# jolibrain/jolineedle

Measured on AMD Instinct MI355X. Metric: glimpse-patches/sec (448px, seq-len 20) REINFORCE step, higher is better.
Workload: dtype f32; 1 GPU; configs[2]/[3]: REINFORCE rollout, gpt-nano + yolox-nano encoder, 448px, seq-len 20, --enable-stop, 64 agents/GPU x 1 GPU, 4480x4480 synthetic images, forced non-STOP actions (S=T); global_batch=64, seq_len=20

## Files before the change

include/jnroll.h:

```cpp
#ifndef JNROLL_H
#define JNROLL_H

#include <stddef.h>
#include <stdint.h>

#ifdef __cplusplus
extern "C" {
#endif

#define JN_ABI_VERSION 2

enum {
  JN_OK = 0,
  JN_EINVAL = -1,
  JN_ENOMEM = -2,
  JN_EHIP = -3,
  JN_ENOTFOUND = -4,
  JN_ESTATE = -5
};

enum { JN_MODE_GREEDY = 0, JN_MODE_SAMPLE = 1, JN_MODE_FORCED = 2 };

enum { JN_NET_GPT_BACKBONE = 0, JN_NET_DETECTOR = 1 };

// ... 117 lines not shown
int jn_gather_patches_views(const jn_image_view* views_dev, int n_views, const int64_t* image_index_dev,
                            const int64_t* positions_dev, void* out_dev, int out_u8, int N, int Hc, int Wc, int P,
                            void* stream);

#define JN_AUG_NPARAM 20
int jn_augment_patches(const float* in_dev, float* out_dev, const float* params_dev, const float* noise_dev,
                       uint64_t seed, int N, int P, void* stream);

int jn_backbone_forward(jn_ctx* ctx, int net, const float* patches_dev, int N, int train,
                        float* fpn0_dev, float* fpn1_dev, float* fpn2_dev, void* stream);
int jn_read_tensor(jn_ctx* ctx, const char* name, float* host_out, size_t numel);
int jn_embed_patches(jn_ctx* ctx, const float* patches_dev, int N, float* out_dev, void* stream);
int jn_zero_grad(jn_ctx* ctx, void* stream);
int jn_backbone_backward(jn_ctx* ctx, int net, const float* patches_dev, int N, const float* g0_dev,
                         const float* g1_dev, const float* g2_dev, void* stream);
typedef struct jn_train_opts {
  int32_t struct_size;
  int32_t reward_norm;
  float ret_mean, ret_std;
  float entropy_weight;
  float loss_scale;
} jn_train_opts;

int jn_reinforce_step(jn_ctx* ctx, int mode, const int64_t* forced_actions_dev,
                      const int64_t* start_positions_dev, uint64_t seed, int stop_early,
                      const jn_train_opts* opts, const jn_rollout_out* out, float* metrics_dev, void* stream);
int jn_reinforce_forward(jn_ctx* ctx, int mode, const int64_t* forced_actions_dev, const int64_t* start_positions_dev,
                         uint64_t seed, int stop_early, const jn_rollout_out* out, void* stream);
int jn_reinforce_backward(jn_ctx* ctx, const float* dlogprobs_dev, const float* dentropies_dev, void* stream);
int jn_arena_segment(jn_ctx* ctx, const char* name, size_t* off, size_t* numel);
// ... 53 lines not shown
```

jolineedle_amd/_lib.py:

```python
import ctypes as C
import os
from pathlib import Path

_LIB = None
LIB_PATH = Path(__file__).resolve().parent / "lib" / "libjnroll.so"

JN_MODE_GREEDY, JN_MODE_SAMPLE, JN_MODE_FORCED = 0, 1, 2
JN_NET_GPT_BACKBONE, JN_NET_DETECTOR = 0, 1


class LibraryNotBuilt(RuntimeError):
    pass


class JnError(RuntimeError):
    pass


class JnConfig(C.Structure):
    _fields_ = [("struct_size", C.c_int32), ("device", C.c_int32),
                ("n_layer", C.c_int32), ("n_head", C.c_int32), ("n_embd", C.c_int32),
                ("block_size", C.c_int32), ("n_actions", C.c_int32), ("patch_size", C.c_int32),
                ("use_pos_emb", C.c_int32), ("no_patch_emb", C.c_int32), ("concat_emb", C.c_int32),
                ("decoder_pos_encoding", C.c_int32), ("pos_emb_size", C.c_int32),
# ... 108 lines not shown
    "jn_set_profiling": (C.c_int, [C.c_void_p, C.c_int]),
    "jn_detector_step": (C.c_int, [C.c_void_p, C.c_void_p, C.c_int, C.c_void_p, C.c_int, C.c_float, C.c_void_p, C.c_void_p]),
    "jn_detector_forward": (C.c_int, [C.c_void_p, C.c_void_p, C.c_int, C.c_void_p, C.c_int, C.c_int, C.c_int, C.c_void_p,
                                      C.c_void_p, C.c_void_p, C.c_void_p, C.c_void_p, C.c_void_p, C.c_void_p]),
    "jn_detector_backward": (C.c_int, [C.c_void_p, C.c_int, C.c_void_p, C.c_float, C.c_void_p]),
    "jn_optimizer_step_group": (C.c_int, [C.c_void_p, C.c_int, C.c_float, C.c_float, C.c_float, C.c_float, C.c_void_p]),
    "jn_reinforce_forward": (C.c_int, [C.c_void_p, C.c_int, C.c_void_p, C.c_void_p, C.c_uint64, C.c_int,
                                       C.POINTER(JnRolloutOut), C.c_void_p]),
    "jn_reinforce_backward": (C.c_int, [C.c_void_p, C.c_void_p, C.c_void_p, C.c_void_p]),
    "jn_arena_segment": (C.c_int, [C.c_void_p, C.c_char_p, C.POINTER(C.c_size_t), C.POINTER(C.c_size_t)]),
    "jn_export_arena": (C.c_int, [C.c_void_p, C.c_int, C.c_void_p, C.c_size_t, C.c_int, C.c_void_p]),
    "jn_import_arena": (C.c_int, [C.c_void_p, C.c_int, C.c_void_p, C.c_size_t, C.c_void_p]),
    "jn_set_dropout": (C.c_int, [C.c_void_p, C.c_float, C.c_uint64]),
    "jn_set_freeze": (C.c_int, [C.c_void_p, C.c_int]),
    "jn_optimizer_steps": (C.c_int, [C.c_void_p, C.c_int, C.POINTER(C.c_int), C.c_int]),
}


def load_library(path=None):
    global _LIB
    if _LIB is not None and path is None:
        return _LIB
    p = Path(path or os.environ.get("JNROLL_LIB", LIB_PATH))
    if not p.exists():
        raise LibraryNotBuilt(
            f"{p} not found: the HIP extension is not built. Run `bash jolineedle_amd/csrc/build.sh` "
            "(or __graft_entry__.build()). There is no CPU fallback for this path.")
    lib = C.CDLL(str(p))
    for name, (res, args) in SIGNATURES.items():
        fn = getattr(lib, name)
# ... 22 lines not shown
```

jolineedle_amd/csrc/api.hip:

```cpp
#include <algorithm>
#include <cmath>
#include <cstdarg>
#include <cstring>
#include <memory>
#include <set>

#include "jn_internal.h"

namespace jnr {

static thread_local char g_err[512] = "";

void set_error(const char* fmt, ...) {
  va_list ap;
  va_start(ap, fmt);
  vsnprintf(g_err, sizeof(g_err), fmt, ap);
  va_end(ap);
}

int build_pafpn(Net& net, std::vector<ParamEntry>& params, const std::string& prefix, float depth, float width,
                bool depthwise, int P);
int build_head(Net& net, std::vector<ParamEntry>& params, const std::string& prefix, float width, bool depthwise,
               int num_classes);

// ... 913 lines not shown
  }
  return JN_OK;
}

static inline float* grad_of(const jn_ctx* ctx, const float* param) { return ctx->grads + (param - ctx->params); }

static int ensure_aux_stream(jn_ctx* ctx) {
  if (ctx->aux_stream) return JN_OK;
  JN_HIP(hipStreamCreateWithFlags(&ctx->aux_stream, hipStreamNonBlocking));
  JN_HIP(hipEventCreateWithFlags(&ctx->aux_fork, hipEventDisableTiming));
  JN_HIP(hipEventCreateWithFlags(&ctx->aux_join, hipEventDisableTiming));
  return JN_OK;
}

static int run_net_backward(jn_ctx* ctx, int ni, int N, const StemSrc& ss, int slot, hipStream_t s, int nsl = 1,
                            long long pos_slot_stride = 0, bool with_head = false, int fpn_zero = 0) {
  Net& net = ctx->nets[ni];
  const int MB = ctx->cfg.max_batch;
  JN_CHECK(nsl >= 1 && nsl <= net.g_slots && slot + nsl <= net.n_slots, JN_ESTATE, "backward over %d slots from %d: not allocated", nsl, slot);
  std::vector<BwdStep> plan;
  int rc = plan_backward(net, with_head, fpn_zero, plan);
  if (rc) return rc;
  JN_HIP(hipMemsetAsync(net.bred, 0, (size_t)nsl * JN_NREP * 2 * net.stat_channels * sizeof(double), s));
  const long long rep_stride = 2LL * net.stat_channels;
  SlotBatch sb;
  sb.n = nsl;
  sb.act = (long long)net.per_image_floats * MB;
  sb.grad = (long long)net.per_image_floats * MB;
  sb.tab = 3LL * net.tab_channels;
  sb.save = 2LL * net.stat_channels;
  sb.red = (long long)JN_NREP * 2 * net.stat_channels;
  sb.consts = 3LL * net.stat_channels;
  sb.pos = pos_slot_stride;
  float* save = slot_save(net, slot);
  auto ptr = [&](const View& v) { return view_ptr(net, slot, MB, v); };
  auto gptr = [&](const View& v) { return net.gact + net.buf_off[v.buf] * (size_t)MB + v.coff; };
  auto tab = [&](const View& v) { return view_tab(net, slot, v); };
  auto ld = [&](const View& v) { return net.bufs[v.buf].C; };
  auto sums = [&](int p, int half) {
    const ConvW& pcw = net.convs[net.ops[p].wslot];
    return net.bred + 2 * (pcw.stat_off + (half > 0 ? pcw.cout / 2 : 0));
  };
  const ChanTab ident{ctx->ident, ctx->ident + 2048, ctx->ident + 4096};
  static const bool no_aux = std::getenv("JN_NO_AUX_STREAM") != nullptr;
  static const bool dbg_plan = std::getenv("JN_DBG_BWD_PLAN") != nullptr;
  bool aux_used = false;
  if (!no_aux) { int ra = ensure_aux_stream(ctx); if (ra) return ra; }
  const int n_ops_b = (int)plan.size();
  static const bool bwd_profile = std::getenv("JN_BWD_PROFILE") != nullptr;
  std::vector<hipEvent_t> bev;
  if (bwd_profile) {
    bev.resize(n_ops_b + 1);
    for (auto& e : bev) (void)hipEventCreate(&e);
    (void)hipEventRecord(bev[n_ops_b], s);
  }
  for (int obi = n_ops_b - 1; obi >= 0; --obi) {
    const Op& op = net.ops[obi];
    const BwdStep& st = plan[obi];
    if (op.wslot >= 0) {
      const ConvW& cw = net.convs[op.wslot];
      float* const gp_out = gptr(st.g);
      const int gld_out = ld(st.g);
      const long long M = (long long)N * op.out.H * op.out.W;
      double* red = net.bred + 2 * cw.stat_off;
      float* consts = net.bconsts + 3 * cw.stat_off;
      const bool pair_halves = st.red_by && !cw.prefix2.empty();
      if (dbg_plan) {
        const int hm = st.red_by;
        const long long sep = pair_halves ? (M / N) * (cw.cout / 2) * (2 - ((hm & 1) + ((hm >> 1) & 1))) : hm ? 0 : (M / N) * cw.cout;
        std::fprintf(stderr, "[bwd-plan] %-34s kind %d cout %4d cin %4d M/patch %6lld stride %d acc_in %d separate-reduce elements/patch %8lld%s\n",
                     op.name.c_str(), (int)op.kind, cw.cout, cw.cin, M / N, op.stride, (int)op.acc_in, sep,
                     pair_halves ? (hm == 3 ? " (both halves by their consumers)" : " (one half by its consumer)") : "");
      }
      if (pair_halves) {
        const int h = cw.cout / 2;
        for (int half = 0; half < 2; ++half) {
          const int c0 = half * h;
          ChanTab ot = tab(op.out);
          ot.sc += c0; ot.sh += c0; ot.fl += c0;
          if (!(st.red_by & (1 << half)))
            launch_bn_bwd_reduce(gp_out + c0, gld_out, (const float*)ptr(op.out) + c0, net.act_dtype, ld(op.out), ot,
                                 save + 2 * (cw.stat_off + c0), h, M, red + 2 * c0, rep_stride, s, sb);
          launch_bn_bwd_consts(red + 2 * c0, rep_stride, (double)M, cw.gamma_dev + c0, cw.beta_dev + c0, save + 2 * (cw.stat_off + c0), consts + 3 * c0,
                               grad_of(ctx, cw.gamma_dev) + c0, grad_of(ctx, cw.beta_dev) + c0, h, s, sb, (st.red_by >> half) & 1);
        }
      } else {
        if (!st.red_by)
// ... 28 lines not shown
            const ChanTab zt = tab(co.out);
            fa.red2_z = (const float*)ptr(co.out); fa.red2_ld = ld(co.out); fa.red2_sc = zt.sc; fa.red2_sh = zt.sh;
          }
          launch_pw_bwd_fused(fa, s);
        }
      } else if (st.route == BR_DW_FUSED) {
        DwBwdFusedArgs fa{};
        fa.g = gp_out; fa.g_ld = gld_out; fa.z = (const float*)ptr(op.out); fa.z_ld = ld(op.out); fa.ot = tab(op.out);
        fa.save = save + 2 * cw.stat_off; fa.consts = consts;
        fa.x = (const float*)ptr(op.in); fa.x_ld = ld(op.in); fa.it = tab(op.in); fa.w = cw.w_dev;
        fa.gin = gptr(op.in); fa.gin_ld = ld(op.in); fa.accumulate = op.acc_in ? 1 : 0; fa.gw = gw; fa.wpart = ctx->wpart;
        fa.C = cw.cout; fa.H = op.in.H; fa.W = op.in.W; fa.OH = op.out.H; fa.OW = op.out.W; fa.N = N; fa.stride = op.stride;
        fa.sb = sb;
        if (st.red_in >= 0) {
          fa.red_in = sums(st.red_in, st.red_half); fa.red_rep_stride = rep_stride;
          fa.accumulate = 0;
        }
        launch_dw_bwd_fused(fa, s);
      } else if (st.route == BR_STEM_FUSED) {
        StemArgs a{ss.src, ss.positions, ss.pos_stride, ss.sample_stride, ss.chan_stride, ss.row_stride, net.P, N, cw.cout,
                   cw.w_dev, nullptr, 0, JN_F32, nullptr, 0, nullptr, 0, 0, ss.src_u8};
        launch_stem_bwd_weight(a, gp_out, gld_out, gw, ctx->wpart, s, sb, (const float*)ptr(op.out), ld(op.out),
                               tab(op.out), save + 2 * cw.stat_off, consts);
      } else {
        launch_bn_bwd_gz(gp_out, gld_out, ptr(op.out), net.act_dtype, ld(op.out), tab(op.out), save + 2 * cw.stat_off, consts,
                         cw.cout, M, s, sb);
        if (st.route == BR_PW) {
          ConvArgs a{};
          a.in = gp_out; a.in_ld = gld_out; a.in_dtype = JN_F32; a.itab = ident; a.w = cw.w_dev; a.bias = nullptr;
          a.out = gptr(op.in); a.out_ld = ld(op.in); a.out_dtype = JN_F32; a.bf16_mfma = net.act_dtype == JN_BF16;
          a.N = N; a.H = op.out.H; a.W = op.out.W; a.OH = op.out.H; a.OW = op.out.W;
// ... 1187 lines not shown
  launch_pw_bwd_weight(e, K, dpe, JN_F32, C, ident, grad_of(ctx, g.efpn_lin_wt), nullptr, Mr, K, C, s);
  launch_colsum_add(dpe, Mr, C, grad_of(ctx, g.efpn_lin_b), s);
  SlotBatch sb;
  sb.n = g_n; sb.act = g_slot; sb.grad = g_slot; sb.tab = 3LL * net.tab_channels;
  ConvArgs a{};
  a.in = ctx->de_ws; a.in_ld = C; a.in_dtype = JN_F32; a.itab = ident; a.w = g.efpn_w; a.bias = nullptr;
  a.out = net.gact + net.buf_off[f2.buf] * (size_t)MB + f2.coff; a.out_ld = net.bufs[f2.buf].C; a.out_dtype = JN_F32; a.bf16_mfma = 0;
  a.N = rows; a.H = f2.H; a.W = f2.W; a.OH = f2.H; a.OW = f2.W; a.cin = C; a.cout = f2.C; a.stride = 1; a.act = ACT_NONE;
  a.accumulate = 0; a.w_transposed = 1; a.in_identity = 1;
  a.n_slots = g_n; a.in_slot_stride = (long long)rows * K; a.out_slot_stride = g_slot; a.tab_slot_stride = 0;
  const bool detached = ctx->enc_net == JN_NET_DETECTOR;
  if (!detached) launch_pw(a, s);
  launch_pw_bwd_weight(ctx->de_ws, C, view_ptr(net, slot, MB, f2), net.act_dtype, net.bufs[f2.buf].C, view_tab(net, slot, f2),
                       grad_of(ctx, g.efpn_w), ctx->wpart, (long long)rows * HW, C, f2.C, s, sb, (long long)rows * K);
  if (detached) return JN_OK;
  for (int i = 0; i < 2; ++i) {
    const View& f = net.fpn[i];
    for (int j = 0; j < g_n; ++j)
      JN_HIP(hipMemsetAsync(net.gact + (size_t)j * g_slot + net.buf_off[f.buf] * (size_t)MB + f.coff, 0,
                            (size_t)rows * f.H * f.W * f.C * sizeof(float), s));
  }
  return run_net_backward(ctx, ctx->enc_net, rows, ss, slot, s, g_n, pos_slot_stride, false, 0x3);
}

}
static int reinforce_backward_impl(jn_ctx* ctx, const jn_rollout_out* out, int S, int stop_early, hipStream_t s);
static int check_train_outputs(jn_ctx* ctx, const jn_rollout_out* out) {
  JN_CHECK(out->logits_dev && out->actions_dev && out->returns_dev && out->logit_masks_dev && out->positions_dev &&
               out->final_emb_dev && out->rewards_dev && out->masks_dev,
           JN_EINVAL, "training needs logits/actions/returns/logit_masks/positions/final_emb/rewards/masks outputs");
  JN_CHECK(!ctx->cfg.no_patch_emb, JN_ESTATE, "training without a patch encoder is not supported");
  JN_CHECK(ctx->cfg.block_size <= 62, JN_EINVAL, "training supports block_size <= 62");
  JN_CHECK(ctx->cfg.act_dtype == JN_F32, JN_ESTATE, "training needs act_dtype = fp32 (bf16 is the inference mode)");
  return JN_OK;
}
extern "C" {

// ... 258 lines not shown

int jn_export_arena(jn_ctx* ctx, int what, float* dst_dev, size_t numel, int accumulate, void* stream) {
  return arena_copy(ctx, what, dst_dev, numel, 1, accumulate, stream);
}

int jn_import_arena(jn_ctx* ctx, int what, const float* src_dev, size_t numel, void* stream) {
  return arena_copy(ctx, what, const_cast<float*>(src_dev), numel, 0, 0, stream);
}

int jn_set_freeze(jn_ctx* ctx, int freeze_detector_backbone) {
  JN_CHECK(ctx, JN_EINVAL, "null ctx");
  ctx->freeze_det_backbone = freeze_detector_backbone != 0;
  return JN_OK;
}

int jn_optimizer_steps(jn_ctx* ctx, int group, int* steps, int set) {
  JN_CHECK(ctx && steps && (group == 0 || group == 1), JN_EINVAL, "jn_optimizer_steps: bad argument");
  int& st = group == 0 ? ctx->adam_step : ctx->adam_step_yolox;
  if (set) st = *steps; else *steps = st;
  return JN_OK;
}

int jn_set_dropout(jn_ctx* ctx, float p, uint64_t seed) {
  JN_CHECK(ctx && p >= 0.0f && p < 1.0f, JN_EINVAL, "dropout probability must be in [0, 1)");
  ctx->pdrop = p; ctx->drop_seed = seed; ctx->drop_ctr = 0;
  return JN_OK;
}

int jn_read_param(jn_ctx* ctx, const char* name, float* host_out, size_t numel) {
  JN_CHECK(ctx && name && host_out && ctx->params, JN_EINVAL, "jn_read_param: bad argument");
// ... 52 lines not shown
```

jolineedle_amd/csrc/jn_internal.h:

```cpp
#pragma once
#include <hip/hip_runtime.h>

#include <cstdint>
#include <cstdio>
#include <map>
#include <string>
#include <vector>

#include "../../include/jnroll.h"
#include "jn_kernels.h"

namespace jnr {

void set_error(const char* fmt, ...);

#define JN_HIP(call)                                                                      \
  do {                                                                                    \
    hipError_t e_ = (call);                                                               \
    if (e_ != hipSuccess) {                                                               \
      jnr::set_error("%s failed: %s (%s:%d)", #call, hipGetErrorString(e_), __FILE__, __LINE__); \
      return JN_EHIP;                                                                     \
    }                                                                                     \
  } while (0)

// ... 98 lines not shown

enum BwdRoute {
  BR_NONE = 0,
  BR_PW_FUSED, BR_PW_FUSED_HALVES,
  BR_DW_FUSED, BR_STEM_FUSED,
  BR_PW, BR_DW, BR_STEM, BR_CONV3_S1, BR_CONV3_S2,
  BR_ADDACT_COPY, BR_ADDACT_FOLD,
  BR_SPP, BR_UPSAMPLE,
};
struct BwdStep {
  BwdRoute route = BR_NONE;
  View g;
  int red_by = 0;
  int red_in = -1, red_half = -1, red_in2 = -1, red_half2 = -1, red_split = 0;
  bool red2 = false;
  int fold = -1;
};
int plan_backward(const Net& net, bool with_head, int fpn_zero, std::vector<BwdStep>& plan);

struct ParamEntry {
  jn_param_info info;
};

struct ParamSeg {
  std::string name;
  int kind = 0, d0 = 0, d1 = 0, d2 = 0;
  size_t off = 0, numel = 0;
};

struct GptW {
  float *wte = nullptr, *wpe = nullptr, *embed_class = nullptr;
  float *proj_wt = nullptr, *proj_b = nullptr;
  float *pos1d = nullptr;
// ... 113 lines not shown
```

jolineedle_amd/csrc/kernels_bwd.hip:

```cpp
#include <hip/hip_runtime.h>

#include <algorithm>
#include <cstdlib>
#include <type_traits>

#include "jn_kernels.h"
#include "jn_reduce.h"
#include "jn_types.h"

namespace jnr {

__device__ __forceinline__ float sigmoidf_(float v) { return __builtin_amdgcn_rcpf(1.0f + __expf(-v)); }
__device__ __forceinline__ float silu_(float v) { return v * sigmoidf_(v); }
__device__ __forceinline__ float dsilu_(float y) {
  const float s = sigmoidf_(y);
  return s * (1.0f + y * (1.0f - s));
}
__device__ __forceinline__ f32x4 tf4_(f32x4 z, f32x4 sc, f32x4 sh, f32x4 fl) {
  f32x4 r;
  r.x = fl.x != 0.0f ? silu_(fmaf(z.x, sc.x, sh.x)) : z.x;
  r.y = fl.y != 0.0f ? silu_(fmaf(z.y, sc.y, sh.y)) : z.y;
  r.z = fl.z != 0.0f ? silu_(fmaf(z.z, sc.z, sh.z)) : z.z;
  r.w = fl.w != 0.0f ? silu_(fmaf(z.w, sc.w, sh.w)) : z.w;
  return r;
// ... 888 lines not shown
  if (nb > cap) nb = cap;
  const dim3 blocks((unsigned)nb, sb.n);
  const size_t smem = (size_t)9 * C * sizeof(float);
#define JN_DWW(S_, T_)                                                                                            \
  hipLaunchKernelGGL((dw_bwd_weight_kernel<S_, T_>), blocks, dim3(256), smem, s, gz, g_ld, (const T_*)x, x_ld, it, \
                     gw, rep, C, H, W, OH, OW, N, sb)
  if (x_dtype == JN_BF16) { if (stride == 1) JN_DWW(1, bf16_t); else JN_DWW(2, bf16_t); }
  else { if (stride == 1) JN_DWW(1, float); else JN_DWW(2, float); }
#undef JN_DWW
  if (rep) launch_wpart_reduce(gw_final, wpart, 9 * C, s);
  return 0;
}

constexpr int DF_TW = 16;

template <int S, int CB, int DF_TH, bool RED>
__global__ __launch_bounds__(256) __attribute__((amdgpu_waves_per_eu(3))) void dw_bwd_fused_kernel(
    const float* __restrict__ g, int g_ld, const float* __restrict__ z, int z_ld, ChanTab ot,
    const float* __restrict__ save, const float* __restrict__ consts, const float* __restrict__ x, int x_ld,
    ChanTab it, const float* __restrict__ w, float* __restrict__ gin, int gin_ld, int accumulate,
    float* __restrict__ gw, int rep, int C, int H, int W, int OH, int OW, int tiles_x, int tiles_y, int n_tiles,
    SlotBatch sb, double* __restrict__ red_in, long long red_rep_stride) {
  constexpr int Q = CB / 4, PS = S == 1 ? CB : CB + JN_DW_S2_PAD;
  constexpr int GH = S == 1 ? DF_TH + 2 : DF_TH + 1, GW = S == 1 ? DF_TW + 2 : DF_TW + 1;
  constexpr int AH = S == 1 ? DF_TH + 2 : 2 * DF_TH + 1, AW = S == 1 ? DF_TW + 2 : 2 * DF_TW + 1;
  constexpr int GROUPS = 256 / (DF_TW * Q), RPG = DF_TH / GROUPS;
  static_assert(RPG >= 1 && RPG * GROUPS == DF_TH, "tile / thread mapping");
  extern __shared__ __attribute__((aligned(16))) float sm[];
  float* Gs = sm;
  float* As = Gs + GH * GW * PS;
  float* red = As + AH * AW * PS;
// ... 25 lines not shown
  f32x4 r1 = {0.f, 0.f, 0.f, 0.f}, r2 = {0.f, 0.f, 0.f, 0.f};
  auto reduce_in = [&](const f32x4& zv, const f32x4& dx) {
    const f32x4 i_sc = JN_C4(7), i_sh = JN_C4(8);
#pragma unroll
    for (int k = 0; k < 4; ++k) {
      const float yv = fmaf(zv[k], i_sc[k], i_sh[k]);
      const float gy = dx[k] * dsilu_(yv);
      r1[k] += gy;
      r2[k] += gy * yv;
    }
  };
  const int xx = (tid / Q) % DF_TW, grp = tid / (Q * DF_TW), j0 = grp * RPG;
  const int wg = blockIdx.x / ncb, n_wg = gridDim.x / ncb;
  constexpr bool OWNER = S == 2 && RED;
  static_assert(!OWNER || RPG == 1, "owner staging: one output pixel per thread and tile");
  f32x4 zraw[OWNER ? 4 : 1];
  for (int tile = wg; tile < n_tiles; tile += n_wg) {
    const int tx = tile % tiles_x, ty = (tile / tiles_x) % tiles_y, n = tile / (tiles_x * tiles_y);
    const int oy0 = ty * DF_TH, ox0 = tx * DF_TW;
    const int gy0 = S == 1 ? oy0 - 1 : oy0, gx0 = S == 1 ? ox0 - 1 : ox0;
    const int ay0 = oy0 * S - 1, ax0 = ox0 * S - 1;
    __syncthreads();
    for (int i = tid; i < GH * GW * Q; i += 256) {
      const int p = i / Q, r = p / GW, cx = p - r * GW;
      const int oy = gy0 + r, ox = gx0 + cx;
      f32x4 v = {0.f, 0.f, 0.f, 0.f};
      if (oy >= 0 && oy < OH && ox >= 0 && ox < OW) {
        const long long pix = ((long long)n * OH + oy) * OW + ox;
        const f32x4 gv = *reinterpret_cast<const f32x4*>(g + pix * g_ld + c);
        const f32x4 zv = *reinterpret_cast<const f32x4*>(z + pix * z_ld + c);
// ... 34 lines not shown
        const int p = i / Q, r = p / AW, cx = p - r * AW;
        const int iy = ay0 + r, ix = ax0 + cx;
        f32x4 v = {0.f, 0.f, 0.f, 0.f};
        if (iy >= 0 && iy < H && ix >= 0 && ix < W)
          v = tf4_(*reinterpret_cast<const f32x4*>(x + (((long long)n * H + iy) * W + ix) * x_ld + c), JN_C4(7), JN_C4(8), JN_C4(9));
        *reinterpret_cast<f32x4*>(As + p * PS + 4 * q) = v;
      }
    }
    __syncthreads();
#pragma unroll 1
    for (int j = 0; j < RPG; ++j) {
      const int y = j0 + j;
      if (S == 1) {
        const f32x4 gc = *reinterpret_cast<const f32x4*>(Gs + ((y + 1) * GW + xx + 1) * PS + 4 * q);
        f32x4 zin = {0.f, 0.f, 0.f, 0.f};
        if (RED && oy0 + y < H && ox0 + xx < W)
          zin = *reinterpret_cast<const f32x4*>(x + (((long long)n * H + oy0 + y) * W + ox0 + xx) * x_ld + c);
        f32x4 acc = {0.f, 0.f, 0.f, 0.f};
#pragma unroll
        for (int ky = 0; ky < 3; ++ky)
#pragma unroll
          for (int kx = 0; kx < 3; ++kx) {
            acc += *reinterpret_cast<const f32x4*>(Gs + ((y + 2 - ky) * GW + xx + 2 - kx) * PS + 4 * q) * JN_C4(10 + ky * 3 + kx);
            dw[ky * 3 + kx] += gc * *reinterpret_cast<const f32x4*>(As + ((y + ky) * AW + xx + kx) * PS + 4 * q);
          }
        const int iy = oy0 + y, ix = ox0 + xx;
        if (iy < H && ix < W) {
          float* op = gin + (((long long)n * H + iy) * W + ix) * gin_ld + c;
          if (RED) reduce_in(zin, acc);
          if (accumulate) acc += *reinterpret_cast<const f32x4*>(op);
          *reinterpret_cast<f32x4*>(op) = acc;
        }
      } else {
        const f32x4 g00 = *reinterpret_cast<const f32x4*>(Gs + (y * GW + xx) * PS + 4 * q);
        const f32x4 g01 = *reinterpret_cast<const f32x4*>(Gs + (y * GW + xx + 1) * PS + 4 * q);
        const f32x4 g10 = *reinterpret_cast<const f32x4*>(Gs + ((y + 1) * GW + xx) * PS + 4 * q);
        const f32x4 g11 = *reinterpret_cast<const f32x4*>(Gs + ((y + 1) * GW + xx + 1) * PS + 4 * q);
#pragma unroll
        for (int ky = 0; ky < 3; ++ky)
#pragma unroll
          for (int kx = 0; kx < 3; ++kx)
            dw[ky * 3 + kx] += g00 * *reinterpret_cast<const f32x4*>(As + ((2 * y + ky) * AW + 2 * xx + kx) * PS + 4 * q);
#pragma unroll
        for (int d = 0; d < 4; ++d) {
          const int iy = 2 * (oy0 + y) + (d >> 1), ix = 2 * (ox0 + xx) + (d & 1);
          if (iy < H && ix < W) {
            float* op = gin + (((long long)n * H + iy) * W + ix) * gin_ld + c;
            f32x4 v;
            if (d == 0) v = g00 * JN_C4(14);
            else if (d == 1) v = g01 * JN_C4(13) + g00 * JN_C4(15);
            else if (d == 2) v = g10 * JN_C4(11) + g00 * JN_C4(17);
            else v = g11 * JN_C4(10) + g10 * JN_C4(12) + g01 * JN_C4(16) + g00 * JN_C4(18);
            if constexpr (OWNER) reduce_in(zraw[d], v);
            if (accumulate) v += *reinterpret_cast<const f32x4*>(op);
            *reinterpret_cast<f32x4*>(op) = v;
          }
        }
      }
    }
  }
  const int lane = tid & 63;
#pragma unroll
  for (int t = 0; t < 9; ++t)
#pragma unroll
    for (int k = 0; k < 4; ++k) {
      float v = dw[t][k];
      for (int off = Q; off < 64; off <<= 1) v += __shfl_xor(v, off);
      if (lane < Q) atomicAdd(&red[t * CB + 4 * q + k], v);
    }
// ... 1 lines not shown
#pragma unroll
    for (int k = 0; k < 4; ++k) {
      float a = r1[k], b = r2[k];
      for (int off = Q; off < 64; off <<= 1) { a += __shfl_xor(a, off); b += __shfl_xor(b, off); }
      if (lane < Q) { atomicAdd(&red[9 * CB + 2 * (4 * q + k)], a); atomicAdd(&red[9 * CB + 2 * (4 * q + k) + 1], b); }
    }
  }
  __syncthreads();
  float* dst = (rep ? gw + ((wg + 5 * blockIdx.y) % JN_NREP) * JN_WPART_MAX : gw);
  for (int i = tid; i < 9 * CB; i += 256) atomicAdd(&dst[(i / CB) * C + cb * CB + (i % CB)], red[i]);
  if (RED)
    if (tid < 2 * CB) atomicAdd(&red_in[(wg % JN_NREP) * red_rep_stride + 2 * cb * CB + tid], (double)red[9 * CB + tid]);
#undef JN_C4
}

template <int S, int CB, int DF_TH, bool RED>
static void launch_dw_bwd_fused_r(const DwBwdFusedArgs& a, hipStream_t s) {
  constexpr int PS = S == 1 ? CB : CB + JN_DW_S2_PAD;
  constexpr int GH = S == 1 ? DF_TH + 2 : DF_TH + 1, GW = S == 1 ? DF_TW + 2 : DF_TW + 1;
  constexpr int AH = S == 1 ? DF_TH + 2 : 2 * DF_TH + 1, AW = S == 1 ? DF_TW + 2 : 2 * DF_TW + 1;
  const size_t smem = ((size_t)(GH * GW + AH * AW) * PS + 11 * CB + 19 * CB) * sizeof(float);
  const int tiles_x = (a.OW + DF_TW - 1) / DF_TW, tiles_y = (a.OH + DF_TH - 1) / DF_TH;
  const int n_tiles = tiles_x * tiles_y * a.N, ncb = a.C / CB;
  int n_wg = 1536 / (ncb * a.sb.n);
  if (n_wg < 8) n_wg = 8;
  if (n_wg > n_tiles) n_wg = n_tiles;
  const int rep = (a.wpart && 9 * a.C <= JN_WPART_MAX) ? 1 : 0;
  hipLaunchKernelGGL((dw_bwd_fused_kernel<S, CB, DF_TH, RED>), dim3((unsigned)(n_wg * ncb), a.sb.n), dim3(256), smem, s, a.g, a.g_ld, a.z,
                     a.z_ld, a.ot, a.save, a.consts, a.x, a.x_ld, a.it, a.w, a.gin, a.gin_ld, a.accumulate,
                     rep ? a.wpart : a.gw, rep, a.C, a.H, a.W, a.OH, a.OW, tiles_x, tiles_y, n_tiles, a.sb, a.red_in,
                     a.red_rep_stride);
  if (rep) launch_wpart_reduce(a.gw, a.wpart, 9 * a.C, s);
}

template <int S, int CB, int DF_TH>
static void launch_dw_bwd_fused_t(const DwBwdFusedArgs& a, hipStream_t s) {
  if (a.red_in) launch_dw_bwd_fused_r<S, CB, DF_TH, true>(a, s);
  else launch_dw_bwd_fused_r<S, CB, DF_TH, false>(a, s);
}

bool dw_bwd_fused_supported(int C, int H, int W, int OH, int OW, int stride) {
  if (C % 16) return false;
  return stride == 1 ? (OH == H && OW == W) : (stride == 2 && OH == (H + 1) / 2 && OW == (W + 1) / 2);
}

int launch_dw_bwd_fused(const DwBwdFusedArgs& a, hipStream_t s) {
  if (a.stride == 1) { if (a.C % 32 == 0) launch_dw_bwd_fused_t<1, 32, 8>(a, s); else launch_dw_bwd_fused_t<1, 16, 8>(a, s); }
  else launch_dw_bwd_fused_t<2, 16, 4>(a, s);
  return 0;
}

constexpr int SB_TY = 8, SB_TX = 32, SB_IH = 2 * SB_TY + 4, SB_IW = 2 * SB_TX + 4;
// ... 460 lines not shown
```

jolineedle_amd/csrc/plan.cpp:

```cpp
#include <cmath>
#include <cstring>

#include "jn_internal.h"

namespace jnr {

namespace {

struct Builder {
  Net& net;
  std::vector<ParamEntry>& params;
  std::string mod_prefix;

  int new_buf(int H, int W, int C) {
    Buf b; b.H = H; b.W = W; b.C = C;
    net.bufs.push_back(b);
    return (int)net.bufs.size() - 1;
  }
  View full(int buf) const {
    const Buf& b = net.bufs[buf];
    View v; v.buf = buf; v.H = b.H; v.W = b.W; v.C = b.C; v.coff = 0;
    return v;
  }
  static View slice(View v, int coff, int C) { v.coff += coff; v.C = C; return v; }
// ... 300 lines not shown

int bn_producer(const Net& net, const View& seg, int reader, int also, int fpn_zero, int* half) {
  *half = -1;
  const int p = sole_writer(net, seg, reader, fpn_zero, [&](int j, bool res) { return j == reader || (res && j == also); });
  if (p < 0) return -1;
  const Op& po = net.ops[p];
  if (po.wslot < 0 || po.out.buf != seg.buf || views_overlap(po.alias, seg)) return -1;
  const ConvW& pw = net.convs[po.wslot];
  if (!pw.has_bn) return -1;
  if (pw.prefix2.empty()) return po.out.coff == seg.coff && po.out.C == seg.C && pw.cout == seg.C ? p : -1;
  if (pw.cout != 2 * seg.C || 2 * pw.cout_first != pw.cout || po.out.C != 2 * seg.C) return -1;
  *half = seg.coff == po.out.coff ? 0 : seg.coff == po.out.coff + seg.C ? 1 : -1;
  return *half >= 0 ? p : -1;
}

int shortcut_sum_conv(const Net& net, const View& seg, int reader, int also, int fpn_zero) {
  const int add = sole_writer(net, seg, reader, fpn_zero, [&](int j, bool res) { return j == reader || (res && j == also); });
  if (add < 0 || net.ops[add].kind != OP_ADDACT) return -1;
  const Op& ao = net.ops[add];
  if (ao.out.coff != seg.coff || ao.out.C != seg.C || ao.in.C != seg.C) return -1;
  const int conv = shortcut_conv(net, add, fpn_zero);
  if (conv < 0) return -1;
  const Op& co = net.ops[conv];
  const ConvW& cw = net.convs[co.wslot];
  return co.kind == OP_PW && !views_overlap(co.alias, ao.in) && cw.has_bn && cw.prefix2.empty() && cw.cout == seg.C ? conv : -1;
}

}

int plan_backward(const Net& net, bool with_head, int fpn_zero, std::vector<BwdStep>& plan) {
  const int n = (with_head || net.n_backbone_ops < 0) ? (int)net.ops.size() : net.n_backbone_ops;
  const bool f32 = net.act_dtype == JN_F32;
  plan.assign(n, BwdStep{});
  auto fused_whole = [&](int j) {
    const Op& o = net.ops[j];
    const ConvW& cw = net.convs[o.wslot];
    return o.kind == OP_PW && f32 && cw.prefix2.empty() && pw_bwd_fused_supported(cw.cout, cw.cin);
  };
  for (int i = n - 1; i >= 0; --i) {
    const Op& op = net.ops[i];
    BwdStep& st = plan[i];
    if (op.wslot >= 0) {
// ... 12 lines not shown
          st.red_in = r2; st.red2 = true; st.red_split = op.in.C;
        } else if (st.red_in < 0 && op.in.C % 32 == 0 && st.fold < 0) {
          const int hC = op.in.C / 2;
          st.red_in = bn_producer(net, seg(0, hC), i, -1, fpn_zero, &st.red_half);
          st.red_in2 = bn_producer(net, seg(hC, hC), i, -1, fpn_zero, &st.red_half2);
          if (st.red_in < 0 && (r2 = shortcut_sum_conv(net, seg(0, hC), i, -1, fpn_zero)) >= 0) {
            st.red_in = r2; st.red2 = true;
          }
          if (st.red_in >= 0 || st.red_in2 >= 0) st.red_split = hC;
        }
      } else if (op.kind == OP_DW && f32 && dw_bwd_fused_supported(cw.cout, op.in.H, op.in.W, op.out.H, op.out.W, op.stride)) {
        st.route = BR_DW_FUSED;
        bool ext_zero = false;
        for (int k = 0; k < 3; ++k) ext_zero = ext_zero || (((fpn_zero >> k) & 1) && views_overlap(op.in, net.fpn[k]));
        if (!op.acc_in || ext_zero) st.red_in = bn_producer(net, op.in, i, -1, fpn_zero, &st.red_half);
      } else if (op.kind == OP_STEM) {
        st.route = f32 ? BR_STEM_FUSED : BR_STEM;
      } else if (op.kind == OP_PW) {
        st.route = BR_PW;
      } else if (op.kind == OP_DW) {
        st.route = BR_DW;
      } else {
        JN_CHECK(op.kind == OP_CONV3, JN_ESTATE, "backward of op %s is not implemented", op.name.c_str());
        st.route = op.stride == 1 ? BR_CONV3_S1 : BR_CONV3_S2;
      }
      continue;
    }
    if (op.kind == OP_ADDACT) {
      const int z = shortcut_conv(net, i, fpn_zero);
      JN_CHECK(op.acc_in || z >= 0, JN_ESTATE, "backward plan: shortcut %s has no single conv behind its input", op.name.c_str());
// ... 5 lines not shown
        if (conv1 >= 0 || res || j > i || o.kind != OP_PW || o.in.buf != op.res.buf || o.in.coff != op.res.coff || o.in.C != op.res.C)
          return false;
        conv1 = j;
        return true;
      }) >= 0;
      const bool fold = f32 && !op.acc_res && one_reader && conv1 >= 0 && net.ops[conv1].acc_in && fused_whole(conv1) &&
                        z >= 0 && fused_whole(z);
      if (fold) plan[conv1].fold = i;
      st.route = fold ? BR_ADDACT_FOLD : BR_ADDACT_COPY;
    } else if (op.kind == OP_SPP) {
      st.route = BR_SPP;
    } else if (op.kind == OP_UPSAMPLE) {
      st.route = BR_UPSAMPLE;
    }
  }
  for (int c = n - 1; c >= 0; --c) {
    const BwdStep& st = plan[c];
    const int runs[2][2] = {{st.red_in, st.red_half}, {st.red_in2, st.red_half2}};
    for (const auto& r : runs) {
      if (r[0] < 0) continue;
      const Op& po = net.ops[r[0]];
      const int bit = r[1] < 0 ? 1 : 1 << r[1];
      JN_CHECK((st.route == BR_PW_FUSED || st.route == BR_DW_FUSED) && r[0] < c && po.wslot >= 0 &&
               (r[1] >= 0) == !net.convs[po.wslot].prefix2.empty() && !(plan[r[0]].red_by & bit),
               JN_ESTATE, "backward plan: %s cannot form the BatchNorm sums of %s", net.ops[c].name.c_str(), po.name.c_str());
      plan[r[0]].red_by |= bit;
    }
    JN_CHECK(st.fold < 0 || st.route == BR_PW_FUSED, JN_ESTATE, "backward plan: shortcut %s folded into %s, not a fused 1x1 conv",
             st.fold < 0 ? "" : net.ops[st.fold].name.c_str(), net.ops[c].name.c_str());
  }
  return JN_OK;
}

}
```

Before: 13120 glimpse-patches/s.

## Fold BatchNorm sums into accumulating depthwise backward and skip redundant FPN gradient zero-fills

Adds an accumulating variant of the fused depthwise-conv backward kernel (RACC). When the op is the last reader of a BN-producing conv, it adds the previously accumulated input gradient and then forms the BatchNorm reduction sums in the same pass, removing a separate reduce pass over that activation. It also replaces the unconditional per-slot memsets of the FPN gradient views with a plan-driven 2D memset, issued only when no fused step fully overwrites the view. A plan-statistics API and a shared plan-checker refactor are added for testing. The risk is correctness of the accumulate ordering and of the analysis that decides which views need no zero-fill.

```diff
diff --git a/include/jnroll.h b/include/jnroll.h
--- a/include/jnroll.h
+++ b/include/jnroll.h
@@ -155,6 +155,8 @@
 int jn_zero_grad(jn_ctx* ctx, void* stream);
 int jn_backbone_backward(jn_ctx* ctx, int net, const float* patches_dev, int N, const float* g0_dev,
                          const float* g1_dev, const float* g2_dev, void* stream);
+int jn_backward_plan_stats(jn_ctx* ctx, int net, int with_head, int fpn_zero, int tamper, long long* reduce_elems,
+                           int* reduce_passes, int* gz_ops, int* fill_mask);
 typedef struct jn_train_opts {
   int32_t struct_size;
   int32_t reward_norm;
diff --git a/jolineedle_amd/_lib.py b/jolineedle_amd/_lib.py
--- a/jolineedle_amd/_lib.py
+++ b/jolineedle_amd/_lib.py
@@ -146,6 +146,8 @@
     "jn_set_dropout": (C.c_int, [C.c_void_p, C.c_float, C.c_uint64]),
     "jn_set_freeze": (C.c_int, [C.c_void_p, C.c_int]),
     "jn_optimizer_steps": (C.c_int, [C.c_void_p, C.c_int, C.POINTER(C.c_int), C.c_int]),
+    "jn_backward_plan_stats": (C.c_int, [C.c_void_p, C.c_int, C.c_int, C.c_int, C.c_int, C.POINTER(C.c_longlong),
+                                         C.POINTER(C.c_int), C.POINTER(C.c_int), C.POINTER(C.c_int)]),
 }
 
 
diff --git a/jolineedle_amd/csrc/api.hip b/jolineedle_amd/csrc/api.hip
--- a/jolineedle_amd/csrc/api.hip
+++ b/jolineedle_amd/csrc/api.hip
@@ -951,7 +951,7 @@
 }
 
 static int run_net_backward(jn_ctx* ctx, int ni, int N, const StemSrc& ss, int slot, hipStream_t s, int nsl = 1,
-                            long long pos_slot_stride = 0, bool with_head = false, int fpn_zero = 0) {
+                            long long pos_slot_stride = 0, bool with_head = false, int fpn_zero = 0, bool fill_unseeded = false) {
   Net& net = ctx->nets[ni];
   const int MB = ctx->cfg.max_batch;
   JN_CHECK(nsl >= 1 && nsl <= net.g_slots && slot + nsl <= net.n_slots, JN_ESTATE, "backward over %d slots from %d: not allocated", nsl, slot);
@@ -959,6 +959,16 @@
   int rc = plan_backward(net, with_head, fpn_zero, plan);
   if (rc) return rc;
   JN_HIP(hipMemsetAsync(net.bred, 0, (size_t)nsl * JN_NREP * 2 * net.stat_channels * sizeof(double), s));
+  const int fill = fill_unseeded ? backward_fpn_fill(net, plan, fpn_zero) : 0;
+  static const bool dbg_plan = std::getenv("JN_DBG_BWD_PLAN") != nullptr;
+  if (dbg_plan) std::fprintf(stderr, "[bwd-fill] zero-filled FPN gradient views: mask 0x%x of unseeded 0x%x\n", fill, fill_unseeded ? fpn_zero : 0);
+  for (int i = 0; i < 3; ++i) {
+    if (!((fill >> i) & 1)) continue;
+    const View& f = net.fpn[i];
+    JN_CHECK(f.coff == 0 && f.C == net.bufs[f.buf].C, JN_ESTATE, "FPN output %d is a channel slice: no contiguous fill", i);
+    JN_HIP(hipMemset2DAsync(net.gact + net.buf_off[f.buf] * (size_t)MB, (size_t)net.per_image_floats * MB * sizeof(float), 0,
+                            (size_t)N * f.H * f.W * f.C * sizeof(float), (size_t)nsl, s));
+  }
   const long long rep_stride = 2LL * net.stat_channels;
   SlotBatch sb;
   sb.n = nsl;
@@ -980,7 +990,6 @@
   };
   const ChanTab ident{ctx->ident, ctx->ident + 2048, ctx->ident + 4096};
   static const bool no_aux = std::getenv("JN_NO_AUX_STREAM") != nullptr;
-  static const bool dbg_plan = std::getenv("JN_DBG_BWD_PLAN") != nullptr;
   bool aux_used = false;
   if (!no_aux) { int ra = ensure_aux_stream(ctx); if (ra) return ra; }
   const int n_ops_b = (int)plan.size();
@@ -1004,10 +1013,11 @@
       const bool pair_halves = st.red_by && !cw.prefix2.empty();
       if (dbg_plan) {
         const int hm = st.red_by;
-        const long long sep = pair_halves ? (M / N) * (cw.cout / 2) * (2 - ((hm & 1) + ((hm >> 1) & 1))) : hm ? 0 : (M / N) * cw.cout;
-        std::fprintf(stderr, "[bwd-plan] %-34s kind %d cout %4d cin %4d M/patch %6lld stride %d acc_in %d separate-reduce elements/patch %8lld%s\n",
+        const long long sep = separate_reduce_elems(net, plan, obi, nullptr);
+        std::fprintf(stderr, "[bwd-plan] %-34s kind %d cout %4d cin %4d M/patch %6lld stride %d acc_in %d separate-reduce elements/patch %8lld%s%s\n",
                      op.name.c_str(), (int)op.kind, cw.cout, cw.cin, M / N, op.stride, (int)op.acc_in, sep,
-                     pair_halves ? (hm == 3 ? " (both halves by their consumers)" : " (one half by its consumer)") : "");
+                     pair_halves ? (hm == 3 ? " (both halves by their consumers)" : " (one half by its consumer)") : "",
+                     st.red_acc ? " (sums its input's producer after accumulating)" : "");
       }
       if (pair_halves) {
         const int h = cw.cout / 2;
@@ -1066,7 +1076,7 @@
         fa.sb = sb;
         if (st.red_in >= 0) {
           fa.red_in = sums(st.red_in, st.red_half); fa.red_rep_stride = rep_stride;
-          fa.accumulate = 0;
+          fa.accumulate = st.red_acc ? 1 : 0;
         }
         launch_dw_bwd_fused(fa, s);
       } else if (st.route == BR_STEM_FUSED) {
@@ -2284,13 +2294,7 @@
   launch_pw_bwd_weight(ctx->de_ws, C, view_ptr(net, slot, MB, f2), net.act_dtype, net.bufs[f2.buf].C, view_tab(net, slot, f2),
                        grad_of(ctx, g.efpn_w), ctx->wpart, (long long)rows * HW, C, f2.C, s, sb, (long long)rows * K);
   if (detached) return JN_OK;
-  for (int i = 0; i < 2; ++i) {
-    const View& f = net.fpn[i];
-    for (int j = 0; j < g_n; ++j)
-      JN_HIP(hipMemsetAsync(net.gact + (size_t)j * g_slot + net.buf_off[f.buf] * (size_t)MB + f.coff, 0,
-                            (size_t)rows * f.H * f.W * f.C * sizeof(float), s));
-  }
-  return run_net_backward(ctx, ctx->enc_net, rows, ss, slot, s, g_n, pos_slot_stride, false, 0x3);
+  return run_net_backward(ctx, ctx->enc_net, rows, ss, slot, s, g_n, pos_slot_stride, false, 0x3, true);
 }
 
 }
@@ -2579,6 +2583,41 @@
   return JN_OK;
 }
 
+int jn_backward_plan_stats(jn_ctx* ctx, int net, int with_head, int fpn_zero, int tamper, long long* reduce_elems,
+                           int* reduce_passes, int* gz_ops, int* fill_mask) {
+  JN_CHECK(ctx && (net == JN_NET_DETECTOR || net == JN_NET_GPT_BACKBONE) && ctx->has_net[net], JN_EINVAL,
+           "jn_backward_plan_stats: no such network");
+  JN_CHECK(fpn_zero >= 0 && fpn_zero < 8 && tamper >= 0 && tamper <= 1, JN_EINVAL, "jn_backward_plan_stats: bad argument");
+  const Net& n = ctx->nets[net];
+  JN_CHECK(!with_head || n.n_backbone_ops >= 0, JN_EINVAL, "jn_backward_plan_stats: the network has no head");
+  std::vector<BwdStep> plan;
+  int rc = plan_backward(n, with_head != 0, fpn_zero, plan);
+  if (rc) return rc;
+  if (tamper) {
+    int first = -1, second = -1;
+    for (int i = (int)plan.size() - 1; i >= 0 && second < 0; --i) {
+      if (plan[i].red_in < 0) continue;
+      if (first < 0) first = i; else second = i;
+    }
+    JN_CHECK(second >= 0, JN_EINVAL, "jn_backward_plan_stats: the plan has fewer than two summing consumers");
+    plan[second].red_in = plan[first].red_in; plan[second].red_half = plan[first].red_half;
+    if ((rc = check_backward_plan(n, plan))) return rc;
+  }
+  long long el = 0;
+  int passes = 0, gz = 0;
+  for (int i = 0; i < (int)plan.size(); ++i) {
+    int np = 0;
+    el += separate_reduce_elems(n, plan, i, &np);
+    passes += np;
+    gz += backward_step_launches_gz(n, plan, i) ? 1 : 0;
+  }
+  if (reduce_elems) *reduce_elems = el;
+  if (reduce_passes) *reduce_passes = passes;
+  if (gz_ops) *gz_ops = gz;
+  if (fill_mask) *fill_mask = backward_fpn_fill(n, plan, fpn_zero);
+  return JN_OK;
+}
+
 int jn_optimizer_steps(jn_ctx* ctx, int group, int* steps, int set) {
   JN_CHECK(ctx && steps && (group == 0 || group == 1), JN_EINVAL, "jn_optimizer_steps: bad argument");
   int& st = group == 0 ? ctx->adam_step : ctx->adam_step_yolox;
diff --git a/jolineedle_amd/csrc/jn_internal.h b/jolineedle_amd/csrc/jn_internal.h
--- a/jolineedle_amd/csrc/jn_internal.h
+++ b/jolineedle_amd/csrc/jn_internal.h
@@ -136,9 +136,14 @@
   int red_by = 0;
   int red_in = -1, red_half = -1, red_in2 = -1, red_half2 = -1, red_split = 0;
   bool red2 = false;
+  bool red_acc = false;
   int fold = -1;
 };
 int plan_backward(const Net& net, bool with_head, int fpn_zero, std::vector<BwdStep>& plan);
+int check_backward_plan(const Net& net, std::vector<BwdStep>& plan);
+long long separate_reduce_elems(const Net& net, const std::vector<BwdStep>& plan, int i, int* passes);
+bool backward_step_launches_gz(const Net& net, const std::vector<BwdStep>& plan, int i);
+int backward_fpn_fill(const Net& net, const std::vector<BwdStep>& plan, int fpn_zero);
 
 struct ParamEntry {
   jn_param_info info;
diff --git a/jolineedle_amd/csrc/kernels_bwd.hip b/jolineedle_amd/csrc/kernels_bwd.hip
--- a/jolineedle_amd/csrc/kernels_bwd.hip
+++ b/jolineedle_amd/csrc/kernels_bwd.hip
@@ -926,7 +926,7 @@
 
 constexpr int DF_TW = 16;
 
-template <int S, int CB, int DF_TH, bool RED>
+template <int S, int CB, int DF_TH, bool RED, bool RACC = false>
 __global__ __launch_bounds__(256) __attribute__((amdgpu_waves_per_eu(3))) void dw_bwd_fused_kernel(
     const float* __restrict__ g, int g_ld, const float* __restrict__ z, int z_ld, ChanTab ot,
     const float* __restrict__ save, const float* __restrict__ consts, const float* __restrict__ x, int x_ld,
@@ -982,6 +982,7 @@
   const int wg = blockIdx.x / ncb, n_wg = gridDim.x / ncb;
   constexpr bool OWNER = S == 2 && RED;
   static_assert(!OWNER || RPG == 1, "owner staging: one output pixel per thread and tile");
+  static_assert(!RACC || RED, "RACC is a form of RED");
   f32x4 zraw[OWNER ? 4 : 1];
   for (int tile = wg; tile < n_tiles; tile += n_wg) {
     const int tx = tile % tiles_x, ty = (tile / tiles_x) % tiles_y, n = tile / (tiles_x * tiles_y);
@@ -1046,8 +1047,11 @@
       if (S == 1) {
         const f32x4 gc = *reinterpret_cast<const f32x4*>(Gs + ((y + 1) * GW + xx + 1) * PS + 4 * q);
         f32x4 zin = {0.f, 0.f, 0.f, 0.f};
-        if (RED && oy0 + y < H && ox0 + xx < W)
+        f32x4 gin_old = {0.f, 0.f, 0.f, 0.f};
+        if (RED && oy0 + y < H && ox0 + xx < W) {
           zin = *reinterpret_cast<const f32x4*>(x + (((long long)n * H + oy0 + y) * W + ox0 + xx) * x_ld + c);
+          if constexpr (RACC) gin_old = *reinterpret_cast<const f32x4*>(gin + (((long long)n * H + oy0 + y) * W + ox0 + xx) * gin_ld + c);
+        }
         f32x4 acc = {0.f, 0.f, 0.f, 0.f};
 #pragma unroll
         for (int ky = 0; ky < 3; ++ky)
@@ -1059,8 +1063,13 @@
         const int iy = oy0 + y, ix = ox0 + xx;
         if (iy < H && ix < W) {
           float* op = gin + (((long long)n * H + iy) * W + ix) * gin_ld + c;
-          if (RED) reduce_in(zin, acc);
-          if (accumulate) acc += *reinterpret_cast<const f32x4*>(op);
+          if constexpr (RACC) {
+            acc += gin_old;
+            reduce_in(zin, acc);
+          } else {
+            if (RED) reduce_in(zin, acc);
+            if (accumulate) acc += *reinterpret_cast<const f32x4*>(op);
+          }
           *reinterpret_cast<f32x4*>(op) = acc;
         }
       } else {
@@ -1078,13 +1087,19 @@
           const int iy = 2 * (oy0 + y) + (d >> 1), ix = 2 * (ox0 + xx) + (d & 1);
           if (iy < H && ix < W) {
             float* op = gin + (((long long)n * H + iy) * W + ix) * gin_ld + c;
-            f32x4 v;
+            f32x4 v, gin_old;
+            if constexpr (RACC) gin_old = *reinterpret_cast<const f32x4*>(op);
             if (d == 0) v = g00 * JN_C4(14);
             else if (d == 1) v = g01 * JN_C4(13) + g00 * JN_C4(15);
             else if (d == 2) v = g10 * JN_C4(11) + g00 * JN_C4(17);
             else v = g11 * JN_C4(10) + g10 * JN_C4(12) + g01 * JN_C4(16) + g00 * JN_C4(18);
-            if constexpr (OWNER) reduce_in(zraw[d], v);
-            if (accumulate) v += *reinterpret_cast<const f32x4*>(op);
+            if constexpr (RACC) {
+              v += gin_old;
+              reduce_in(zraw[d], v);
+            } else {
+              if constexpr (OWNER) reduce_in(zraw[d], v);
+              if (accumulate) v += *reinterpret_cast<const f32x4*>(op);
+            }
             *reinterpret_cast<f32x4*>(op) = v;
           }
         }
@@ -1116,7 +1131,7 @@
 #undef JN_C4
 }
 
-template <int S, int CB, int DF_TH, bool RED>
+template <int S, int CB, int DF_TH, bool RED, bool RACC = false>
 static void launch_dw_bwd_fused_r(const DwBwdFusedArgs& a, hipStream_t s) {
   constexpr int PS = S == 1 ? CB : CB + JN_DW_S2_PAD;
   constexpr int GH = S == 1 ? DF_TH + 2 : DF_TH + 1, GW = S == 1 ? DF_TW + 2 : DF_TW + 1;
@@ -1128,7 +1143,7 @@
   if (n_wg < 8) n_wg = 8;
   if (n_wg > n_tiles) n_wg = n_tiles;
   const int rep = (a.wpart && 9 * a.C <= JN_WPART_MAX) ? 1 : 0;
-  hipLaunchKernelGGL((dw_bwd_fused_kernel<S, CB, DF_TH, RED>), dim3((unsigned)(n_wg * ncb), a.sb.n), dim3(256), smem, s, a.g, a.g_ld, a.z,
+  hipLaunchKernelGGL((dw_bwd_fused_kernel<S, CB, DF_TH, RED, RACC>), dim3((unsigned)(n_wg * ncb), a.sb.n), dim3(256), smem, s, a.g, a.g_ld, a.z,
                      a.z_ld, a.ot, a.save, a.consts, a.x, a.x_ld, a.it, a.w, a.gin, a.gin_ld, a.accumulate,
                      rep ? a.wpart : a.gw, rep, a.C, a.H, a.W, a.OH, a.OW, tiles_x, tiles_y, n_tiles, a.sb, a.red_in,
                      a.red_rep_stride);
@@ -1137,7 +1152,8 @@
 
 template <int S, int CB, int DF_TH>
 static void launch_dw_bwd_fused_t(const DwBwdFusedArgs& a, hipStream_t s) {
-  if (a.red_in) launch_dw_bwd_fused_r<S, CB, DF_TH, true>(a, s);
+  if (a.red_in && a.accumulate) launch_dw_bwd_fused_r<S, CB, DF_TH, true, true>(a, s);
+  else if (a.red_in) launch_dw_bwd_fused_r<S, CB, DF_TH, true>(a, s);
   else launch_dw_bwd_fused_r<S, CB, DF_TH, false>(a, s);
 }
 
diff --git a/jolineedle_amd/csrc/plan.cpp b/jolineedle_amd/csrc/plan.cpp
--- a/jolineedle_amd/csrc/plan.cpp
+++ b/jolineedle_amd/csrc/plan.cpp
@@ -338,6 +338,24 @@
   return *half >= 0 ? p : -1;
 }
 
+int bn_producer_last_reader(const Net& net, const View& seg, int reader, int n, int fpn_zero) {
+  int others = 0;
+  const int p = sole_writer(net, seg, reader, fpn_zero, [&](int j, bool res) {
+    if (res) return false;
+    if (j == reader) return true;
+    const Op& o = net.ops[j];
+    const bool covers = o.in.buf == seg.buf && o.in.coff <= seg.coff && o.in.coff + o.in.C >= seg.coff + seg.C;
+    if (j < reader || j >= n || o.wslot < 0 || !covers) return false;
+    ++others;
+    return true;
+  });
+  if (p < 0 || !others) return -1;
+  const Op& po = net.ops[p];
+  if (po.wslot < 0 || po.alias.buf >= 0 || po.out.buf != seg.buf || po.out.coff != seg.coff || po.out.C != seg.C) return -1;
+  const ConvW& pw = net.convs[po.wslot];
+  return pw.has_bn && pw.prefix2.empty() && pw.cout == seg.C ? p : -1;
+}
+
 int shortcut_sum_conv(const Net& net, const View& seg, int reader, int also, int fpn_zero) {
   const int add = sole_writer(net, seg, reader, fpn_zero, [&](int j, bool res) { return j == reader || (res && j == also); });
   if (add < 0 || net.ops[add].kind != OP_ADDACT) return -1;
@@ -350,6 +368,29 @@
   return co.kind == OP_PW && !views_overlap(co.alias, ao.in) && cw.has_bn && cw.prefix2.empty() && cw.cout == seg.C ? conv : -1;
 }
 
+}
+
+int check_backward_plan(const Net& net, std::vector<BwdStep>& plan) {
+  for (auto& st : plan) st.red_by = 0;
+  const int n = (int)plan.size();
+  for (int c = n - 1; c >= 0; --c) {
+    const BwdStep& st = plan[c];
+    const int runs[2][2] = {{st.red_in, st.red_half}, {st.red_in2, st.red_half2}};
+    for (const auto& r : runs) {
+      if (r[0] < 0) continue;
+      const Op& po = net.ops[r[0]];
+      const int bit = r[1] < 0 ? 1 : 1 << r[1];
+      JN_CHECK((st.route == BR_PW_FUSED || st.route == BR_DW_FUSED) && r[0] < c && po.wslot >= 0 &&
+               (r[1] >= 0) == !net.convs[po.wslot].prefix2.empty() && !(plan[r[0]].red_by & bit),
+               JN_ESTATE, "backward plan: %s cannot form the BatchNorm sums of %s", net.ops[c].name.c_str(), po.name.c_str());
+      plan[r[0]].red_by |= bit;
+    }
+    JN_CHECK(!st.red_acc || (st.route == BR_DW_FUSED && st.red_in >= 0 && st.red_half < 0 && net.ops[c].acc_in), JN_ESTATE,
+             "backward plan: %s sums an accumulated gradient it cannot", net.ops[c].name.c_str());
+    JN_CHECK(st.fold < 0 || st.route == BR_PW_FUSED, JN_ESTATE, "backward plan: shortcut %s folded into %s, not a fused 1x1 conv",
+             st.fold < 0 ? "" : net.ops[st.fold].name.c_str(), net.ops[c].name.c_str());
+  }
+  return JN_OK;
 }
 
 int plan_backward(const Net& net, bool with_head, int fpn_zero, std::vector<BwdStep>& plan) {
@@ -392,6 +433,7 @@
         bool ext_zero = false;
         for (int k = 0; k < 3; ++k) ext_zero = ext_zero || (((fpn_zero >> k) & 1) && views_overlap(op.in, net.fpn[k]));
         if (!op.acc_in || ext_zero) st.red_in = bn_producer(net, op.in, i, -1, fpn_zero, &st.red_half);
+        else if ((st.red_in = bn_producer_last_reader(net, op.in, i, n, fpn_zero)) >= 0) st.red_acc = true;
       } else if (op.kind == OP_STEM) {
         st.route = f32 ? BR_STEM_FUSED : BR_STEM;
       } else if (op.kind == OP_PW) {
@@ -427,22 +469,50 @@
       st.route = BR_UPSAMPLE;
     }
   }
-  for (int c = n - 1; c >= 0; --c) {
-    const BwdStep& st = plan[c];
-    const int runs[2][2] = {{st.red_in, st.red_half}, {st.red_in2, st.red_half2}};
-    for (const auto& r : runs) {
-      if (r[0] < 0) continue;
-      const Op& po = net.ops[r[0]];
-      const int bit = r[1] < 0 ? 1 : 1 << r[1];
-      JN_CHECK((st.route == BR_PW_FUSED || st.route == BR_DW_FUSED) && r[0] < c && po.wslot >= 0 &&
-               (r[1] >= 0) == !net.convs[po.wslot].prefix2.empty() && !(plan[r[0]].red_by & bit),
-               JN_ESTATE, "backward plan: %s cannot form the BatchNorm sums of %s", net.ops[c].name.c_str(), po.name.c_str());
-      plan[r[0]].red_by |= bit;
-    }
-    JN_CHECK(st.fold < 0 || st.route == BR_PW_FUSED, JN_ESTATE, "backward plan: shortcut %s folded into %s, not a fused 1x1 conv",
-             st.fold < 0 ? "" : net.ops[st.fold].name.c_str(), net.ops[c].name.c_str());
-  }
-  return JN_OK;
-}
-
-}
+  return check_backward_plan(net, plan);
+}
+
+long long separate_reduce_elems(const Net& net, const std::vector<BwdStep>& plan, int i, int* passes) {
+  const Op& op = net.ops[i];
+  if (passes) *passes = 0;
+  if (op.wslot < 0) return 0;
+  const ConvW& cw = net.convs[op.wslot];
+  const long long px = (long long)op.out.H * op.out.W;
+  const int hm = plan[i].red_by;
+  int np = hm ? 0 : 1;
+  long long el = hm ? 0 : px * cw.cout;
+  if (hm && !cw.prefix2.empty()) {
+    np = 2 - ((hm & 1) + ((hm >> 1) & 1));
+    el = px * (cw.cout / 2) * np;
+  }
+  if (passes) *passes = np;
+  return el;
+}
+
+bool backward_step_launches_gz(const Net& net, const std::vector<BwdStep>& plan, int i) {
+  const BwdRoute r = plan[i].route;
+  return net.ops[i].wslot >= 0 && (r == BR_PW || r == BR_DW || r == BR_STEM || r == BR_CONV3_S1 || r == BR_CONV3_S2);
+}
+
+int backward_fpn_fill(const Net& net, const std::vector<BwdStep>& plan, int fpn_zero) {
+  int fill = 0;
+  for (int k = 0; k < 3; ++k) {
+    if (!((fpn_zero >> k) & 1)) continue;
+    const View& f = net.fpn[k];
+    bool written = false;
+    for (int j = (int)plan.size() - 1; j >= 0; --j) {
+      const Op& o = net.ops[j];
+      if (!views_overlap(o.in, f) && !views_overlap(o.res, f) && !views_overlap(o.out, f) && !views_overlap(o.alias, f) &&
+          !(o.kind == OP_SPP && o.out.buf == f.buf))
+        continue;
+      const BwdStep& st = plan[j];
+      written = st.route == BR_DW_FUSED && st.red_in >= 0 && !st.red_acc && o.in.buf == f.buf && o.in.coff == f.coff &&
+                o.in.C == f.C && !views_overlap(o.out, f);
+      break;
+    }
+    if (!written) fill |= 1 << k;
+  }
+  return fill;
+}
+
+}
```

Result: no change. 13230 glimpse-patches/s (median of 6 runs) (+0.8%).
